# RazonIn4K/image-restoration-platform

Measured on AMD Instinct MI355X. Metric: restored images/sec @1024x1024 bs=8, higher is better.
Workload: dtype bf16; 1 GPU; 1024x1024 RGB u8, batch 8 per GPU: fused classifier scan + RestoreNet-v0 (43 convs, 779.9 GFLOP/image), seeded random-init weights; global_batch=8, parallelism=per-image data parallel x1, no collective, streams=1

## Files before the change

image_restoration_platform_amd/build.py:

```python
import concurrent.futures
import os
import subprocess
import sys

HERE = os.path.dirname(os.path.abspath(__file__))
CSRC = os.path.join(HERE, "csrc")
OBJ = os.path.join(HERE, "build")
LIB = os.path.join(HERE, "lib", "libire.so")

SOURCES = [
    ("classifier.hip", ["-ffp-contract=off"] + (["-DCLS_ABL=" + os.environ["CLS_ABL"]] if os.environ.get("CLS_ABL") else [])),
    ("conv_mfma.hip", []),
    ("conv_rb.hip", (["-DIRE_RB_ABLATE"] if os.environ.get("IRE_RB_ABLATE") else []) +
     (["-DIRE_RB_NGP64=" + os.environ["IRE_RB_NGP64"]] if os.environ.get("IRE_RB_NGP64") else [])),
    ("conv_w4.hip", (["-DIRE_W4_STAMPS"] if os.environ.get("IRE_RB_ABLATE") else []) +
     (["-DIRE_W4_TICKS"] if os.environ.get("IRE_RB_ABLATE") == "2" else []) +
     (["-DW4_TEPI=" + os.environ["IRE_W4_TEPI"]] if os.environ.get("IRE_W4_TEPI") else []) +
     (["-DIRE_W4_TL"] if os.environ.get("IRE_W4_TL") else [])),
    ("conv_up.hip", (["-DIRE_UP_ABL=" + os.environ["IRE_UP_ABL"]] if os.environ.get("IRE_UP_ABL") else []) +
     (["-DIRE_UP_D=" + os.environ["IRE_UP_D"]] if os.environ.get("IRE_UP_D") else []) +
     (["-DIRE_UP_TEPI=" + os.environ["IRE_UP_TEPI"]] if os.environ.get("IRE_UP_TEPI") else [])),
    ("conv_upq.hip", os.environ.get("UQ_DEFS", "").split()),
    ("conv_dnq.hip", os.environ.get("DQ_DEFS", "").split()),
    ("conv_down.hip", (["-DDN_LD_NT=" + os.environ["DN_LD_NT"]] if os.environ.get("DN_LD_NT") else [])),
    ("conv_stem.hip", []),
    ("conv_f8.hip", []),
    ("conv_pc.hip", (["-DC3_ABL=" + os.environ["C3_ABL"]] if os.environ.get("C3_ABL") else []) +
     (["-DC3_PRIO=" + os.environ["C3_PRIO"]] if os.environ.get("C3_PRIO") else []) +
     (["-DC3_RES_PRE=" + os.environ["C3_RES_PRE"]] if os.environ.get("C3_RES_PRE") else []) +
     (["-DC3_TEPI=" + os.environ["C3_TEPI"]] if os.environ.get("C3_TEPI") else []) +
     (["-DC3_TEPI64=" + os.environ["C3_TEPI64"]] if os.environ.get("C3_TEPI64") else []) +
     (["-DIRE_LD_ONCE32=" + os.environ["IRE_LD_ONCE32"]] if os.environ.get("IRE_LD_ONCE32") else []) +
     (["-DC3_PROD8=" + os.environ["C3_PROD8"]] if os.environ.get("C3_PROD8") else []) +
     (["-DIRE_PC_TICKS"] if os.environ.get("IRE_RB_ABLATE") == "2" else []) + (["-DIRE_W4_TL"] if os.environ.get("IRE_W4_TL") else [])),
    ("conv_pk.hip", (["-DPK_ABL=" + os.environ["PK_ABL"]] if os.environ.get("PK_ABL") else []) +
     (["-DPK_TICKS"] if os.environ.get("PK_TICKS") else []) + (["-DIRE_W4_TL"] if os.environ.get("IRE_W4_TL") else []) + os.environ.get("PK_DEFS", "").split()),
    ("gn.hip", []),
    ("fusion.hip", (["-DFUSE_FL=" + os.environ["FUSE_FL"]] if os.environ.get("FUSE_FL") else [])),
    ("preprocess.hip", []),
    ("encode.hip", []),
    ("deflate.hip", []),
    ("jpeg.hip", []),
    ("jpeg_progenc.hip", []),
    ("jpeg_dec.hip", []),
    ("png_dec.hip", []),
    ("icc.hip", []),
    ("codec.cpp", ["--offload-host-only"]),
    ("engine.cpp", []),
    ("strips.cpp", []),
    ("api.cpp", []),
]
COMMON = ["--offload-arch=gfx950", "-O3", "-std=c++17", "-fPIC", "-Wall", "-Wno-unused-function",
          "-D__HIP_PLATFORM_AMD__"] + ([] if os.environ.get("IRE_SLP") == "1" else ["-fno-slp-vectorize"]) + \
         (["-DIRE_ST_LINE=" + os.environ["IRE_ST_LINE"]] if os.environ.get("IRE_ST_LINE") else []) + \
         (["-DIRE_ST_PART=" + os.environ["IRE_ST_PART"]] if os.environ.get("IRE_ST_PART") else []) + \
         (["-DIRE_LD_ONCE=" + os.environ["IRE_LD_ONCE"]] if os.environ.get("IRE_LD_ONCE") else []) + \
         (["-DIRE_LD_IN=" + os.environ["IRE_LD_IN"]] if os.environ.get("IRE_LD_IN") else []) + \
         os.environ.get("IRE_XFLAGS", "").split()

def _hipcc():
    for c in (os.environ.get("HIPCC"), "/opt/rocm/bin/hipcc", "hipcc"):
        if c and (os.path.isabs(c) and os.path.exists(c) or not os.path.isabs(c)):
            return c
    raise RuntimeError("hipcc not found")


def _deps_mtime():
    m = 0.0
    for root, _, files in os.walk(CSRC):
        for f in files:
            if f.endswith((".hpp", ".inc", ".h")):
                m = max(m, os.path.getmtime(os.path.join(root, f)))
    m = max(m, os.path.getmtime(os.path.join(HERE, "..", "include", "ire.h")))
    return m


def _compile(src, extra, force, hdr_m):
    path = os.path.join(CSRC, src)
    obj = os.path.join(OBJ, src.replace(".", "_") + ".o")
    lang = ["-x", "hip"] if src.endswith((".hip", ".cpp")) else []
    cmd = [_hipcc()] + COMMON + extra + lang + ["-c", path, "-o", obj]
    stamp = obj + ".cmd"
    cmd_id = " ".join(cmd).replace(HERE, "<pkg>")
    same_cmd = os.path.exists(stamp) and open(stamp).read() == cmd_id
    if (not force and same_cmd and os.path.exists(obj) and os.path.getmtime(obj) > os.path.getmtime(path)
            and os.path.getmtime(obj) > hdr_m):
        return obj
    r = subprocess.run(cmd, capture_output=True, text=True)
    if r.returncode != 0:
        raise RuntimeError(f"hipcc failed for {src}:\n{r.stderr[-4000:]}")
    with open(stamp, "w") as f:
        f.write(cmd_id)
    return obj


def build(force=False, verbose=False):
    os.makedirs(OBJ, exist_ok=True)
    os.makedirs(os.path.dirname(LIB), exist_ok=True)
    srcs = [(s, f) for s, f in SOURCES if os.path.exists(os.path.join(CSRC, s))]
    if os.path.exists(os.path.join(CSRC, "fusion_stub.cpp")) and not os.path.exists(os.path.join(CSRC, "fusion.hip")):
        srcs.append(("fusion_stub.cpp", []))
    hdr_m = _deps_mtime()
    with concurrent.futures.ThreadPoolExecutor(max_workers=6) as ex:
        objs = list(ex.map(lambda sf: _compile(sf[0], sf[1], force, hdr_m), srcs))
    if force or not os.path.exists(LIB) or any(os.path.getmtime(o) > os.path.getmtime(LIB) for o in objs):
        cmd = [_hipcc(), "--offload-arch=gfx950", "-shared", "-fPIC", "-o", LIB] + objs + ["-lpthread"]
        r = subprocess.run(cmd, capture_output=True, text=True)
        if r.returncode != 0:
            raise RuntimeError(f"link failed:\n{r.stderr[-4000:]}")
    build_node_addon()
    try:
        build_torch_extension()
    except ImportError as e:
        print("build: torch extension skipped (%s)" % e, file=sys.stderr)
    except RuntimeError as e:
        print("build: torch extension NOT built: %s" % str(e)[-1500:], file=sys.stderr)
    if verbose:
        print("built", LIB)
    return LIB


def build_node_addon():
    src = os.path.join(HERE, "node", "ire_napi.cc")
    out = os.path.join(HERE, "node", "ire_napi.node")
    inc = "/usr/include/node"
    if not os.path.exists(os.path.join(inc, "node_api.h")):
        return None
    if os.path.exists(out) and os.path.getmtime(out) > max(os.path.getmtime(src), _deps_mtime()):
        return out
    r = subprocess.run(["g++", "-O2", "-shared", "-fPIC", "-I" + inc, "-DNODE_GYP_MODULE_NAME=ire_napi", src, "-o", out, "-ldl"],
                       capture_output=True, text=True)
    if r.returncode != 0:
        raise RuntimeError("node addon build failed:\n" + r.stderr[-2000:])
    return out


def build_torch_extension():
    src = os.path.join(CSRC, "torch_ext.cpp")
    out = os.path.join(HERE, "lib", "_ire_torch.so")
    import sysconfig
    from torch.utils import cpp_extension as ce
    incs = ce.include_paths() + [sysconfig.get_paths()["include"], "/opt/rocm/include"]
    libdir = ce.library_paths()[0]
    cmd = (["g++", "-O2", "-std=c++17", "-shared", "-fPIC", "-D__HIP_PLATFORM_AMD__", "-DUSE_ROCM", "-DTORCH_EXTENSION_NAME=_ire_torch",
            "-DTORCH_API_INCLUDE_EXTENSION_H", "-D_GLIBCXX_USE_CXX11_ABI=" + str(int(__import__("torch")._C._GLIBCXX_USE_CXX11_ABI))] +
           ["-isystem" + i for i in incs] + [src, "-o", out, "-L" + libdir, "-Wl,-rpath," + libdir,
            "-lc10", "-lc10_hip", "-ltorch_cpu", "-ltorch", "-ltorch_python", "-ldl"])
    stamp = os.path.join(OBJ, "_ire_torch.cmd")
    cmd_id = " ".join(cmd).replace(HERE, "<pkg>")
    if (os.path.exists(out) and os.path.exists(stamp) and open(stamp).read() == cmd_id and
            os.path.getmtime(out) > max(os.path.getmtime(src), os.path.getmtime(os.path.join(HERE, "..", "include", "ire.h")))):
        return out
    r = subprocess.run(cmd, capture_output=True, text=True)
    if r.returncode != 0:
        raise RuntimeError("torch extension build failed:\n" + r.stderr[-3000:])
    os.makedirs(OBJ, exist_ok=True)
    with open(stamp, "w") as f:
        f.write(cmd_id)
    return out


if __name__ == "__main__":
    build(force="--force" in sys.argv, verbose=True)
```

image_restoration_platform_amd/csrc/conv_pc.hip:

```cpp
#include "conv_mfma.hpp"
#include "conv_plan.hpp"
#include "conv_prims.hpp"
#include "gn_fold.hpp"
#include "persist.hpp"

#include <type_traits>

namespace ire {

namespace {

#ifndef C3_RES_PRE
#define C3_RES_PRE -1
#endif
#ifndef C3_SCALAR
#define C3_SCALAR 1
#endif
#ifndef C3_PRIO
#define C3_PRIO 1
#endif
#ifndef C3_TEPI
#define C3_TEPI 1
#endif
#ifndef IRE_LD_ONCE32
#define IRE_LD_ONCE32 2
#endif
#ifndef C3_TEPI64
#define C3_TEPI64 1
#endif
#ifndef C3_PROD8
#define C3_PROD8 0
#endif
#ifndef C3_INTERIOR
#define C3_INTERIOR 0
#endif
#ifndef C3_ABL
#define C3_ABL 0
#endif
constexpr int C3_CONS = 512, C3_PROD = 256, C3_THREADS = C3_CONS + C3_PROD;
constexpr int pc_prod(int C, bool head) { return (C3_PROD8 && C == 32 && !head) ? 512 : 256; }
constexpr int C3_TH = 16, C3_TW = 32, C3_IH = C3_TH + 2, C3_IW = C3_TW + 2;
constexpr int C3_IN_CHUNKS = C3_IH * C3_IW * 4;
constexpr int C3_P_ITERS = (C3_IN_CHUNKS + C3_PROD - 1) / C3_PROD;
constexpr int C3_IN_BYTES = C3_P_ITERS * C3_PROD * 16;
template <int C> struct PcCfg {
    static constexpr int NT = C < 64 ? 32 : 64;
    static constexpr int NBLK = C / NT;
    static constexpr int NKC = C / 32;
    static constexpr int NTL = NT / 32;
    static constexpr int W_STAGE = 36 * NT * 16;
    static constexpr int W_STAGE_CHUNKS = 36 * NT;
    static constexpr int W_LDS = NKC * W_STAGE;
    static constexpr int W_OFF = 2 * C3_IN_BYTES;
    static constexpr int BIAS_OFF = W_OFF + W_LDS;
    static constexpr int NCC = NT / 8;
    static constexpr int RED_OFF = BIAS_OFF + C * 4;
    static constexpr int RED_HALF = 8 * NCC * 4;
    static constexpr int COEF_IMGS = pc_coef_imgs(C);
    static constexpr int COEF_OFF = RED_OFF + 2 * RED_HALF * 4;
    static constexpr int HEAD_OFF = COEF_OFF + COEF_IMGS * C * 2 * 4;
    static constexpr int PATCH_OFF = HEAD_OFF + (C == 32 ? 8 * 2 * 2 * 96 : 0);
    static constexpr int CNT_OFF = PATCH_OFF + (C == 32 ? 8 * 2048 : 0);
    static constexpr int LDS = CNT_OFF + (C == 64 ? 16 : 0);
    static_assert(LDS <= 160 * 1024, "LDS");
};

template <int C, bool RESID, bool HEAD>
__global__ __launch_bounds__(C3_CONS + pc_prod(C, HEAD)) void conv_pc_kernel(ConvArgs a) {
    using K = PcCfg<C>;
    constexpr int PROD = pc_prod(C, HEAD), THREADS = C3_CONS + PROD;
    constexpr int P_ITERS = (C3_IN_CHUNKS + PROD - 1) / PROD;
    static_assert(P_ITERS * PROD * 16 == C3_IN_BYTES, "tile slots");
    constexpr int NKC = K::NKC, NTL = K::NTL, NCC = K::NCC, NT = K::NT;
    static_assert(!HEAD || C == 32, "the head is a C = 32 layer");
    __shared__ __attribute__((aligned(16))) unsigned char smem[K::LDS];
    const int tid = threadIdx.x;
    const int lane = tid & 63, wave = tid >> 6;
    const int r = lane & 31, h = lane >> 5;
    int stamp_item = 0;
    auto stamp = [&](int k) {
#ifdef IRE_PC_TICKS
        const unsigned long long t = __builtin_amdgcn_s_memtime();
        if (a.stamps && lane == 0 && (wave == 0 || wave == 8) && blockIdx.x < 8 && stamp_item < 64)
            a.stamps[(((size_t)blockIdx.x * 2 + (wave ? 1 : 0)) * 64 + stamp_item) * 10 + k] = t;
#else
        (void)k;
#endif
    };

    auto tl = [&](int slot) {
#ifdef IRE_W4_TL
        if (a.stamps && tid == 0) {
            a.stamps[(size_t)blockIdx.x * 32 + slot * 2] = __builtin_amdgcn_s_memrealtime();
            a.stamps[(size_t)blockIdx.x * 32 + slot * 2 + 1] = __builtin_amdgcn_s_memtime();
        }
#else
        (void)slot;
#endif
    };
    const int tiles_per_img = a.tiles_x * a.tiles_y;
    PersistCursor cursor(a.tiles_x, a.tiles_y, a.nimg, K::NBLK, NKC, (int)gridDim.x, (int)blockIdx.x, a.walk_rev != 0);
    const int n_items = cursor.my_items;
    if (n_items == 0) return;
    const int n_stages = n_items * NKC;
    tl(0);
    {
        const unsigned char* ws = reinterpret_cast<const unsigned char*>(a.w);
        const unsigned wl = (unsigned)(size_t)(__attribute__((address_space(3))) unsigned char*)smem + K::W_OFF;
        constexpr int PIECES = NKC * K::W_STAGE_CHUNKS / 64;
        static_assert((NKC * K::W_STAGE_CHUNKS) % 64 == 0, "whole wave-instructions");
        const int wv = __builtin_amdgcn_readfirstlane(wave);
        for (int p = wv; p < PIECES; p += THREADS / 64) glds16(ws + ((size_t)p * 64 + lane) * 16, wl + p * 1024);
    }
    if (a.gn_stats) gn_fold(a, smem, cursor.first_img, cursor.last_img, 512, reinterpret_cast<float2*>(smem + K::COEF_OFF));
    tl(1);

    {
        if (tid < C) reinterpret_cast<float*>(smem + K::BIAS_OFF)[tid] = a.bias[tid];
        if constexpr (C == 64) { if (tid == 0) *reinterpret_cast<unsigned*>(smem + K::CNT_OFF) = 0u; }
        const int nim = cursor.last_img - cursor.first_img + 1;
        const float2* ab = a.ab + (size_t)cursor.first_img * C;
        float2* cd = reinterpret_cast<float2*>(smem + K::COEF_OFF);
        if (!a.gn_stats) for (int i = tid; i < nim * C; i += THREADS) cd[i] = ab[i];
    }
    asm volatile("s_waitcnt vmcnt(0)" ::: "memory");
    __syncthreads();
    tl(2);

    if (__builtin_amdgcn_readfirstlane(wave) >= 8) {
#if C3_PRIO
        if (C3_PRIO != 1 || C != 32 || HEAD) asm volatile("s_setprio %0" :: "n"(C3_PRIO));
#endif
        const int tp = tid - C3_CONS;
        const int c8 = tp & 3;
        int rel[P_ITERS], lds_off[P_ITERS];
        unsigned pyx[P_ITERS];
#pragma unroll
        for (int i = 0; i < P_ITERS; ++i) {
            const int q = tp + i * PROD;
            const int p = q >> 2;
            const int py = p / C3_IW, px = p - py * C3_IW;
            pyx[i] = ((unsigned)py << 8) | (unsigned)px;
            rel[i] = (py * a.Win + px) * (2 * C) + c8 * 16;
            lds_off[i] = (p * 4 + (c8 ^ ((p >> 2) & 3))) * 16;
        }
        uint4 R[P_ITERS];
        unsigned okbits = 0;
        float cA[8], cB[8];
        PersistStage ls = cursor.cur;
        auto load_chunk = [&](int i) __attribute__((always_inline)) {
            const PersistItem& lit = ls.it;
            const int oy1 = lit.ty * C3_TH - 1, ox1 = lit.tx * C3_TW - 1;
            const char* base = reinterpret_cast<const char*>(a.in0) + (size_t)lit.img * a.in_rows * a.Win * (2 * C) + ls.kc * 64;
            const __amdgpu_buffer_rsrc_t irsrc = __builtin_amdgcn_make_buffer_rsrc(const_cast<char*>(base), 0, tensor_bytes(a.in_rows, a.Win, 2 * C) - (unsigned)(ls.kc * 64), 0x00020000);
            const unsigned base_off = (unsigned)((oy1 + a.in_row_off) * a.Win + ox1) * (unsigned)(2 * C);
            const int y_lo = max(a.iy_lo - oy1, 0), y_hi = min(a.iy_lo + a.iy_span - oy1, C3_IH);
            const int x_lo = max(-ox1, 0), x_hi = min(a.Win - ox1, C3_IW);
            const int py = (int)(pyx[i] >> 8), px = (int)(pyx[i] & 0xffu);
            const bool ok = (unsigned)(py - y_lo) < (unsigned)(y_hi - y_lo) && (unsigned)(px - x_lo) < (unsigned)(x_hi - x_lo);
            const unsigned off = ok ? base_off + rel[i] : 0xffffffffu;
            if constexpr (C3_ABL & 8) { R[i] = make_uint4(off, 0x3f803f80u, i, 0x3f803f80u); }
            else {
                const u32x4_t lv = __builtin_amdgcn_raw_buffer_load_b128(irsrc, off, 0, IRE_LD_IN);
                R[i] = make_uint4(lv.x, lv.y, lv.z, lv.w);
            }
            okbits = (okbits & ~(1u << i)) | (ok ? (1u << i) : 0u);
        };
        auto load_coeffs = [&](const PersistStage& st) __attribute__((always_inline)) {
            const float4* ab = reinterpret_cast<const float4*>(smem + K::COEF_OFF) + ((st.it.img - cursor.first_img) * C + st.kc * 32 + c8 * 8) / 2;
#pragma unroll
            for (int e = 0; e < 4; ++e) { const float4 v = ab[e]; cA[2 * e] = v.x; cB[2 * e] = v.y; cA[2 * e + 1] = v.z; cB[2 * e + 1] = v.w; }
        };
        auto transform_stage_v = [&](unsigned char* tile, auto interior_tag) __attribute__((always_inline)) {
            constexpr bool INTERIOR = decltype(interior_tag)::value;
            auto pair = [&](auto pp_tag) __attribute__((always_inline)) {
                constexpr int pp_ = decltype(pp_tag)::value, i = 2 * pp_;
                constexpr int NCH = i + 1 < P_ITERS ? 2 : 1;
                constexpr int NW = 4 * NCH, NV = 8 * NCH;
                constexpr int i1 = NCH == 2 ? i + 1 : i;
                const unsigned wds[8] = {R[i].x, R[i].y, R[i].z, R[i].w, R[i1].x, R[i1].y, R[i1].z, R[i1].w};
                unsigned o[8];
                if constexpr (C3_ABL & 1) {
#pragma unroll
                    for (int w = 0; w < NW; ++w) o[w] = wds[w];
                } else {
#if C3_SCALAR
                    float y[16], e[16];
#pragma unroll
                    for (int w = 0; w < NW; ++w) {
                        const int d = w & 3;
                        y[2 * w] = __builtin_fmaf(bf16_lo(wds[w]), cA[2 * d], cB[2 * d]);
                        y[2 * w + 1] = __builtin_fmaf(bf16_hi(wds[w]), cA[2 * d + 1], cB[2 * d + 1]);
                    }
#pragma unroll
                    for (int k = 0; k < NV; ++k) e[k] = y[k] * (-1.4426950408889634f);
                    __builtin_amdgcn_sched_barrier(0);
#pragma unroll
                    for (int k = 0; k < NV; ++k) e[k] = __builtin_amdgcn_exp2f(e[k]);
                    __builtin_amdgcn_sched_barrier(0);
#pragma unroll
                    for (int k = 0; k < NV; ++k) e[k] = e[k] + 1.0f;
                    __builtin_amdgcn_sched_barrier(0);
#pragma unroll
                    for (int k = 0; k < NV; ++k) e[k] = __builtin_amdgcn_rcpf(e[k]);
                    __builtin_amdgcn_sched_barrier(0);
#pragma unroll
                    for (int w = 0; w < NW; ++w) o[w] = pack_bf16(y[2 * w] * e[2 * w], y[2 * w + 1] * e[2 * w + 1]);
#else
                    static_assert(NCH == 2, "the packed-f32 form handles whole pairs");
                    f32x2_t y[8], e[8];
#pragma unroll
                    for (int w = 0; w < 8; ++w) {
                        const int d = w & 3;
                        const f32x2_t x = {bf16_lo(wds[w]), bf16_hi(wds[w])};
                        const f32x2_t A = {cA[2 * d], cA[2 * d + 1]}, B = {cB[2 * d], cB[2 * d + 1]};
                        y[w] = __builtin_elementwise_fma(x, A, B);
                        e[w] = y[w] * (-1.4426950408889634f);
                    }
                    __builtin_amdgcn_sched_barrier(0);
#pragma unroll
                    for (int w = 0; w < 8; ++w) e[w] = f32x2_t{__builtin_amdgcn_exp2f(e[w].x), __builtin_amdgcn_exp2f(e[w].y)};
                    __builtin_amdgcn_sched_barrier(0);
#pragma unroll
                    for (int w = 0; w < 8; ++w) e[w] = e[w] + 1.0f;
                    __builtin_amdgcn_sched_barrier(0);
#pragma unroll
                    for (int w = 0; w < 8; ++w) e[w] = f32x2_t{__builtin_amdgcn_rcpf(e[w].x), __builtin_amdgcn_rcpf(e[w].y)};
                    __builtin_amdgcn_sched_barrier(0);
#pragma unroll
                    for (int w = 0; w < 8; ++w) { const f32x2_t sv = y[w] * e[w]; o[w] = pack_bf16(sv.x, sv.y); }
#endif
                }
#pragma unroll
                for (int k = 0; k < NCH; ++k) {
                    uint4 ov = make_uint4(o[4 * k], o[4 * k + 1], o[4 * k + 2], o[4 * k + 3]);
                    if constexpr (!INTERIOR) {
                        const unsigned m = (okbits >> (i + k)) & 1u ? 0xffffffffu : 0u;
                        ov = make_uint4(o[4 * k] & m, o[4 * k + 1] & m, o[4 * k + 2] & m, o[4 * k + 3] & m);
                    }
                    *reinterpret_cast<uint4*>(tile + lds_off[i + k]) = ov;
                }
                load_chunk(i);
                if constexpr (NCH == 2) load_chunk(i + 1);
                __builtin_amdgcn_sched_barrier(0);
            };
            pair(std::integral_constant<int, 0>{}); pair(std::integral_constant<int, 1>{}); pair(std::integral_constant<int, 2>{});
            if constexpr (P_ITERS > 6) { pair(std::integral_constant<int, 3>{}); pair(std::integral_constant<int, 4>{}); }
        };
        unsigned past_last = 0u;
        {
            const int q = tp + (P_ITERS - 1) * PROD;
            past_last = (q >> 2) >= C3_IH * C3_IW ? (1u << (P_ITERS - 1)) : 0u;
        }
        auto transform_stage = [&](unsigned char* tile) __attribute__((always_inline)) {
            if constexpr (C3_INTERIOR) {
                if (__builtin_amdgcn_ballot_w64((okbits | past_last) != (1u << P_ITERS) - 1u) == 0) { transform_stage_v(tile, std::true_type{}); return; }
            }
            transform_stage_v(tile, std::false_type{});
        };
#pragma unroll
        for (int i = 0; i < P_ITERS; ++i) load_chunk(i);
        load_coeffs(ls);
        ls = cursor.next();
        transform_stage(smem);
        lds_barrier();
        for (int t = 0; t < n_stages; ++t) {
            stamp_item = t / NKC;
            stamp(3 * (t % NKC) + 0);
            load_coeffs(ls);
            ls = cursor.next();
            transform_stage(smem + ((t + 1) & 1) * C3_IN_BYTES);
            stamp(3 * (t % NKC) + 1);
            lds_barrier();
            stamp(3 * (t % NKC) + 2);
        }
        return;
    }

    int a_off[2][9];
#pragma unroll
    for (int m = 0; m < 2; ++m)
#pragma unroll
        for (int tap = 0; tap < 9; ++tap) {
            const int ky = tap / 3, kx = tap - ky * 3;
            const int p = (wave * 2 + m + ky) * C3_IW + r + kx;
            a_off[m][tap] = (p * 4 + (h ^ ((p >> 2) & 3))) * 16;
        }
    const unsigned char* wb = smem + K::W_OFF + (h * NT + r) * 16;
    const float* bias_lds = reinterpret_cast<const float*>(smem + K::BIAS_OFF);
    f32x16_t bias_acc;
    if constexpr (C == 32) {
#pragma unroll
        for (int i = 0; i < 16; ++i) bias_acc[i] = bias_lds[16 * (i >> 3) + 8 * h + (i & 7)];
    }
    float* red_base = reinterpret_cast<float*>(smem + K::RED_OFF);
    int st_img = -1, st_tile = 0, st_nb = 0, st_par = 0, red_par = 0;
    auto flush_stats = [&]() {
        if (HEAD || st_img < 0) return;
        constexpr int G = C / 8, NGL = NT / G, CPG = G / 8;
        if (tid < NGL) {
            const float* red = red_base + st_par * K::RED_HALF;
            float s = 0.f, q = 0.f;
#pragma unroll
            for (int w = 0; w < 8; ++w) {
                if constexpr (C == 32) {
                    const float* d = red + (w * NCC + (tid >> 1)) * 4 + 2 * (tid & 1);
                    s += d[0]; q += d[1];
                } else {
#pragma unroll
                    for (int k = 0; k < CPG; ++k) {
                        const float* d = red + (w * NCC + tid * CPG + k) * 4;
                        s += d[0] + d[2]; q += d[1] + d[3];
                    }
                }
            }
            float* st = a.stats + (((size_t)st_img * tiles_per_img + st_tile) * 8 + (st_nb * NT) / G + tid) * 2;
            st[0] = s; st[1] = q;
        }
        st_img = -1;
    };

    f32x16_t acc[2][NTL];
    uint4 erv[2 * NTL][2];
    constexpr int RES_WANT = C3_RES_PRE >= 0 ? C3_RES_PRE : (C == 64 ? 1 : 2);
    constexpr int RES_PRE = RES_WANT < 2 * NTL ? RES_WANT : 2 * NTL;
    unsigned eoffs[2];
    bool einb[2];
    constexpr bool TEPI = C3_TEPI && C == 32 && !HEAD;
    constexpr bool TEPI64 = C3_TEPI64 && C == 64 && !HEAD;
    unsigned toffs[2];
    bool trow[2];
    int tcol = 0;
    unsigned hin[2] = {0u, 0u};
    size_t hoff[2] = {0, 0};
    bool hok[2] = {false, false};
    PersistStage cs = cursor.cur;
    int stage_no = 0;
    lds_barrier();
    for (int t = 0; t < n_items; ++t) {
        const PersistItem it = cs.it;
        stamp_item = t;
        stamp(0);
        flush_stats();
        {
            const int oyb = it.ty * C3_TH + wave * 2, ox = it.tx * C3_TW + r;
            const bool colok = ox < a.Wout;
            const int oxc = min(ox, a.Wout - 1);
#pragma unroll
            for (int m = 0; m < 2; ++m) {
                const int oy = oyb + m;
                einb[m] = colok && oy < a.Hout;
                eoffs[m] = ((unsigned)((min(oy, a.Hout - 1) * a.Wout + oxc) * C + it.nb * NT) << 1) + (unsigned)(h * 16);
            }
            if constexpr (TEPI || TEPI64) {
                constexpr int LPP = C / 8;
                tcol = it.tx * C3_TW + lane / LPP;
#pragma unroll
                for (int m = 0; m < 2; ++m) {
                    const int oy = oyb + m;
                    trow[m] = oy < a.Hout;
                    toffs[m] = ((unsigned)((min(oy, a.Hout - 1) * a.Wout + tcol) * C + 8 * (lane % LPP)) << 1);
                }
            }
            if constexpr (RESID && TEPI64 && !(C3_ABL & 64)) {
                char* rbase = const_cast<char*>(reinterpret_cast<const char*>(a.resid)) + (size_t)it.img * a.Hout * a.Wout * (2 * C);
                const __amdgpu_buffer_rsrc_t rrsrc = __builtin_amdgcn_make_buffer_rsrc(rbase, 0, tensor_bytes(a.Hout, a.Wout, 2 * C), 0x00020000);
#pragma unroll
                for (int m = 0; m < 2; ++m)
#pragma unroll
                    for (int k = 0; k < RES_PRE; ++k) {
                        const bool ok = trow[m] && tcol + 8 * k < a.Wout;
                        const u32x4_t v = __builtin_amdgcn_raw_buffer_load_b128(rrsrc, ok ? toffs[m] + (unsigned)(8 * k * 2 * C) : 0xffffffffu, 0, IRE_LD_ONCE32);
                        erv[k][m] = make_uint4(v.x, v.y, v.z, v.w);
                    }
            } else
            if constexpr (RESID && TEPI && !(C3_ABL & 64)) {
                char* rbase = const_cast<char*>(reinterpret_cast<const char*>(a.resid)) + (size_t)it.img * a.Hout * a.Wout * (2 * C);
                const __amdgpu_buffer_rsrc_t rrsrc = __builtin_amdgcn_make_buffer_rsrc(rbase, 0, tensor_bytes(a.Hout, a.Wout, 2 * C), 0x00020000);
#pragma unroll
                for (int m = 0; m < 2; ++m)
#pragma unroll
                    for (int k = 0; k < 2; ++k) {
                        const bool ok = trow[m] && tcol + 16 * k < a.Wout;
                        const u32x4_t v = __builtin_amdgcn_raw_buffer_load_b128(rrsrc, ok ? toffs[m] + (unsigned)(16 * k * 2 * C) : 0xffffffffu, 0, IRE_LD_ONCE);
                        erv[k][m] = make_uint4(v.x, v.y, v.z, v.w);
                    }
            } else if constexpr (RESID && (C3_ABL & 64)) {
#pragma unroll
                for (int g = 0; g < 2 * NTL; ++g)
#pragma unroll
                    for (int m = 0; m < 2; ++m) erv[g][m] = make_uint4(eoffs[m], g, 0x3f803f80u, m);
            } else if constexpr (RESID) {
                const char* rbase = reinterpret_cast<const char*>(a.resid) + (size_t)it.img * a.Hout * a.Wout * (2 * C);
#pragma unroll
                for (int m = 0; m < 2; ++m)
#pragma unroll
                    for (int g = 0; g < RES_PRE; ++g) erv[g][m] = *reinterpret_cast<const uint4*>(rbase + eoffs[m] + (unsigned)(g * 32));
            }
            if constexpr (HEAD) {
                const int vbytes = 3 * min(C3_TW, a.Wout - it.tx * C3_TW);
#pragma unroll
                for (int m = 0; m < 2; ++m) {
                    const int oy = oyb + m;
                    hok[m] = oy < a.Hout && 4 * lane < vbytes;
                    hoff[m] = (((size_t)it.img * a.Hout + min(oy, a.Hout - 1)) * a.Wout + it.tx * C3_TW) * 3 + 4 * (size_t)min(lane, 23);
                    hin[m] = hok[m] ? *reinterpret_cast<const unsigned*>(a.u8_in + hoff[m]) : 0u;
                }
            }
        }
        if constexpr (C != 32) {
#pragma unroll
            for (int j = 0; j < NTL; ++j)
#pragma unroll
                for (int q = 0; q < 4; ++q) {
                    const float4 bv = *reinterpret_cast<const float4*>(bias_lds + it.nb * NT + j * 32 + 16 * (q >> 1) + 8 * h + 4 * (q & 1));
#pragma unroll
                    for (int m = 0; m < 2; ++m) { acc[m][j][4 * q + 0] = bv.x; acc[m][j][4 * q + 1] = bv.y; acc[m][j][4 * q + 2] = bv.z; acc[m][j][4 * q + 3] = bv.w; }
                }
        }
#pragma unroll NKC <= 2 ? NKC : 1
        for (int kc = 0; kc < NKC; ++kc) {
          auto stage_body = [&](auto par_tag) __attribute__((always_inline)) {
            constexpr int PAR = decltype(par_tag)::value;
            const int par = PAR >= 0 ? PAR : (stage_no & 1);
            const unsigned char* ib = smem + par * C3_IN_BYTES;
            const unsigned char* wk = wb + kc * K::W_STAGE;
            bf16x8_t af[2][2], bf[2][NTL];
            auto read_k = [&](int g, bf16x8_t (&pa)[2], bf16x8_t (&pw)[NTL]) __attribute__((always_inline)) {
                const int tap = g >> 1, cp = g & 1;
#pragma unroll
                for (int m = 0; m < 2; ++m) pa[m] = __builtin_bit_cast(bf16x8_t, *reinterpret_cast<const uint4*>(ib + (a_off[m][tap] ^ (cp << 5))));
#pragma unroll
                for (int j = 0; j < NTL; ++j) pw[j] = __builtin_bit_cast(bf16x8_t, *reinterpret_cast<const uint4*>(wk + ((tap * 4 + 2 * cp) * NT + j * 32) * 16));
            };
            read_k(0, af[0], bf[0]);
            if constexpr (!(C3_ABL & 4))
#pragma unroll
            for (int g = 0; g < 18; ++g) {
                if (g + 1 < 18) read_k(g + 1, af[(g + 1) & 1], bf[(g + 1) & 1]);
                __builtin_amdgcn_sched_barrier(0);
#pragma unroll
                for (int m = 0; m < 2; ++m)
#pragma unroll
                    for (int j = 0; j < NTL; ++j) {
                        if constexpr (C == 32) acc[m][j] = __builtin_amdgcn_mfma_f32_32x32x16_bf16(bf[g & 1][j], af[g & 1][m], (kc == 0 && g == 0) ? bias_acc : acc[m][j], 0, 0, 0);
                        else acc[m][j] = __builtin_amdgcn_mfma_f32_32x32x16_bf16(bf[g & 1][j], af[g & 1][m], acc[m][j], 0, 0, 0);
                    }
                __builtin_amdgcn_sched_barrier(0);
            }
          };
            if constexpr (NKC == 1 && HEAD) { if (stage_no & 1) stage_body(std::integral_constant<int, 1>{}); else stage_body(std::integral_constant<int, 0>{}); }
            else if constexpr (NKC == 2) { if (kc & 1) stage_body(std::integral_constant<int, 1>{}); else stage_body(std::integral_constant<int, 0>{}); }
            else stage_body(std::integral_constant<int, -1>{});
            ++stage_no;
            stamp(kc == 0 ? 1 : 3);
            if (kc + 1 < NKC) { cs = cursor.next(); lds_barrier(); stamp(2); }
        }
        if constexpr (RESID && TEPI64 && RES_PRE < 2 * NTL) {
            char* rbase = const_cast<char*>(reinterpret_cast<const char*>(a.resid)) + (size_t)it.img * a.Hout * a.Wout * (2 * C);
            const __amdgpu_buffer_rsrc_t rrsrc = __builtin_amdgcn_make_buffer_rsrc(rbase, 0, tensor_bytes(a.Hout, a.Wout, 2 * C), 0x00020000);
#pragma unroll
            for (int m = 0; m < 2; ++m)
#pragma unroll
                for (int k = RES_PRE; k < 2 * NTL; ++k) {
                    const bool ok = trow[m] && tcol + 8 * k < a.Wout;
                    const u32x4_t v = __builtin_amdgcn_raw_buffer_load_b128(rrsrc, ok ? toffs[m] + (unsigned)(8 * k * 2 * C) : 0xffffffffu, 0, 0);
                    erv[k][m] = make_uint4(v.x, v.y, v.z, v.w);
                }
        } else if constexpr (RESID && RES_PRE < 2 * NTL) {
            const char* rbase = reinterpret_cast<const char*>(a.resid) + (size_t)it.img * a.Hout * a.Wout * (2 * C);
#pragma unroll
            for (int m = 0; m < 2; ++m)
#pragma unroll
                for (int g = RES_PRE; g < 2 * NTL; ++g) erv[g][m] = *reinterpret_cast<const uint4*>(rbase + eoffs[m] + (unsigned)(g * 32));
        }
        if constexpr (HEAD) {
            unsigned char* hp = smem + K::HEAD_OFF + wave * (2 * 2 * 96);
#pragma unroll
            for (int m = 0; m < 2; ++m)
                if (lane < 24) *reinterpret_cast<unsigned*>(hp + m * 96 + 4 * lane) = hin[m];
#pragma unroll
            for (int m = 0; m < 2; ++m) {
                if (h == 0) {
#pragma unroll
                    for (int c = 0; c < 3; ++c) {
                        float vv = (float)hp[m * 96 + 3 * r + c] + acc[m][0][c];
                        vv = fminf(fmaxf(vv, 0.f), 255.f);
                        hp[192 + m * 96 + 3 * r + c] = (unsigned char)(int)floorf(vv + 0.5f);
                    }
                }
            }
#pragma unroll
            for (int m = 0; m < 2; ++m)
                if (hok[m]) *reinterpret_cast<unsigned*>(a.u8_out + hoff[m]) = *reinterpret_cast<const unsigned*>(hp + 192 + m * 96 + 4 * min(lane, 23));
        } else if constexpr (C3_ABL & 2) {
#pragma unroll
            for (int m = 0; m < 2; ++m)
#pragma unroll
                for (int j = 0; j < NTL; ++j) asm volatile("" :: "v"(acc[m][j]));
        } else if constexpr (TEPI64) {
            char* obase = reinterpret_cast<char*>(a.out) + (size_t)it.img * a.Hout * a.Wout * (2 * C);
            const __amdgpu_buffer_rsrc_t orsrc = __builtin_amdgcn_make_buffer_rsrc(obase, 0, tensor_bytes(a.Hout, a.Wout, 2 * C), 0x00020000);
            const bf16x2_t ones = __builtin_bit_cast(bf16x2_t, 0x3f803f80u);
            float* redw = red_base + red_par * K::RED_HALF;
            {
                volatile unsigned* cnt = reinterpret_cast<volatile unsigned*>(smem + K::CNT_OFF);
                asm volatile("s_waitcnt lgkmcnt(0)" ::: "memory");
                if (lane == 0) __hip_atomic_fetch_add(const_cast<unsigned*>(cnt), 1u, __ATOMIC_RELAXED, __HIP_MEMORY_SCOPE_WORKGROUP);
                const unsigned target = 8u * (unsigned)(t + 1);
                while ((unsigned)__builtin_amdgcn_readfirstlane((int)*cnt) < target) __builtin_amdgcn_s_sleep(1);
            }
            unsigned char* patch = smem + C3_IN_BYTES + wave * 4096;
            const int wsw = r & 7;
            const int pq = lane >> 3, cq = lane & 7;
            float sA = 0.f, qA = 0.f;
#pragma unroll
            for (int half = 0; half < 2; ++half)
#pragma unroll
            for (int m = 0; m < 2; ++m) {
#pragma unroll
                for (int g = 0; g < 2 * NTL; ++g) {
                    const f32x16_t& c = acc[m][g >> 1];
                    const int pp = g & 1;
                    const u32x4_t wv = {pack_bf16(c[8 * pp + 0], c[8 * pp + 1]), pack_bf16(c[8 * pp + 2], c[8 * pp + 3]),
                                        pack_bf16(c[8 * pp + 4], c[8 * pp + 5]), pack_bf16(c[8 * pp + 6], c[8 * pp + 7])};
                    *reinterpret_cast<u32x4_t*>(patch + r * 128 + (((2 * g + h) ^ wsw) << 4)) = wv;
                }
#pragma unroll
                for (int k = 2 * half; k < 2 * half + 2; ++k) {
                    const int p = pq + 8 * k;
                    const u32x4_t v = *reinterpret_cast<const u32x4_t*>(patch + p * 128 + ((cq ^ (p & 7)) << 4));
                    unsigned w[4] = {v.x, v.y, v.z, v.w};
                    if constexpr (RESID) {
                        const uint4 rr = erv[k][m];
                        const unsigned rw[4] = {rr.x, rr.y, rr.z, rr.w};
#pragma unroll
                        for (int d = 0; d < 4; ++d) w[d] = pack_bf16(bf16_lo(w[d]) + bf16_lo(rw[d]), bf16_hi(w[d]) + bf16_hi(rw[d]));
                    }
                    const bool ok = trow[m] && tcol + 8 * k < a.Wout;
                    const float mf = ok ? 1.f : 0.f;
                    float ts0 = 0.f, tq0 = 0.f;
                    if constexpr (!(C3_ABL & 32))
#pragma unroll
                    for (int d = 0; d < 4; ++d) {
                        const bf16x2_t bv = __builtin_bit_cast(bf16x2_t, w[d]);
                        ts0 = __builtin_amdgcn_fdot2_f32_bf16(bv, ones, ts0, false); tq0 = __builtin_amdgcn_fdot2_f32_bf16(bv, bv, tq0, false);
                    }
                    sA = __builtin_fmaf(ts0, mf, sA); qA = __builtin_fmaf(tq0, mf, qA);
                    const u32x4_t o4 = {w[0], w[1], w[2], w[3]};
                    if constexpr (C3_ABL & 16) asm volatile("" :: "v"(o4));
                    else __builtin_amdgcn_raw_buffer_store_b128(o4, orsrc, ok ? toffs[m] + (unsigned)(8 * k * 2 * C) : 0xffffffffu, 0, IRE_ST_LINE);
                }
            }
            if constexpr (!(C3_ABL & 32)) {
                float t2[2] = {sA, qA};
#pragma unroll
                for (int k = 0; k < 2; ++k) t2[k] = ror_add<8>(t2[k]);
#pragma unroll
                for (int k = 0; k < 2; ++k) t2[k] = swap16_add(t2[k]);
#pragma unroll
                for (int k = 0; k < 2; ++k) t2[k] = swap32_add(t2[k]);
                if (lane < 8) *reinterpret_cast<float4*>(redw + (wave * NCC + lane) * 4) = make_float4(t2[0], t2[1], 0.f, 0.f);
            }
            st_img = it.img; st_tile = it.tile; st_nb = it.nb; st_par = red_par; red_par ^= 1;
        } else if constexpr (TEPI) {
            char* obase = reinterpret_cast<char*>(a.out) + (size_t)it.img * a.Hout * a.Wout * (2 * C);
            const __amdgpu_buffer_rsrc_t orsrc = __builtin_amdgcn_make_buffer_rsrc(obase, 0, tensor_bytes(a.Hout, a.Wout, 2 * C), 0x00020000);
            const bf16x2_t ones = __builtin_bit_cast(bf16x2_t, 0x3f803f80u);
            float* redw = red_base + red_par * K::RED_HALF;
            unsigned char* patch = smem + K::PATCH_OFF + wave * 2048;
            const int wsw = (r >> 1) & 3;
            const int pq = lane >> 2, cq = lane & 3;
            float sA = 0.f, qA = 0.f, sB = 0.f, qB = 0.f;
#pragma unroll
            for (int m = 0; m < 2; ++m) {
                const f32x16_t& c = acc[m][0];
#pragma unroll
                for (int pp = 0; pp < 2; ++pp) {
                    const u32x4_t wv = {pack_bf16(c[8 * pp + 0], c[8 * pp + 1]), pack_bf16(c[8 * pp + 2], c[8 * pp + 3]),
                                        pack_bf16(c[8 * pp + 4], c[8 * pp + 5]), pack_bf16(c[8 * pp + 6], c[8 * pp + 7])};
                    *reinterpret_cast<u32x4_t*>(patch + r * 64 + (((2 * pp + h) ^ wsw) << 4)) = wv;
                }
#pragma unroll
                for (int k = 0; k < 2; ++k) {
                    const int p = pq + 16 * k;
                    const u32x4_t v = *reinterpret_cast<const u32x4_t*>(patch + p * 64 + ((cq ^ ((p >> 1) & 3)) << 4));
                    unsigned w[4] = {v.x, v.y, v.z, v.w};
                    if constexpr (RESID) {
                        const uint4 rr = erv[k][m];
                        const unsigned rw[4] = {rr.x, rr.y, rr.z, rr.w};
#pragma unroll
                        for (int d = 0; d < 4; ++d) w[d] = pack_bf16(bf16_lo(w[d]) + bf16_lo(rw[d]), bf16_hi(w[d]) + bf16_hi(rw[d]));
                    }
                    const bool ok = trow[m] && tcol + 16 * k < a.Wout;
                    const float mf = ok ? 1.f : 0.f;
                    float ts0 = 0.f, tq0 = 0.f, ts1 = 0.f, tq1 = 0.f;
                    if constexpr (!(C3_ABL & 32))
#pragma unroll
                    for (int d = 0; d < 4; ++d) {
                        const bf16x2_t bv = __builtin_bit_cast(bf16x2_t, w[d]);
                        if (d < 2) { ts0 = __builtin_amdgcn_fdot2_f32_bf16(bv, ones, ts0, false); tq0 = __builtin_amdgcn_fdot2_f32_bf16(bv, bv, tq0, false); }
                        else { ts1 = __builtin_amdgcn_fdot2_f32_bf16(bv, ones, ts1, false); tq1 = __builtin_amdgcn_fdot2_f32_bf16(bv, bv, tq1, false); }
                    }
                    sA = __builtin_fmaf(ts0, mf, sA); qA = __builtin_fmaf(tq0, mf, qA);
                    sB = __builtin_fmaf(ts1, mf, sB); qB = __builtin_fmaf(tq1, mf, qB);
                    const u32x4_t o4 = {w[0], w[1], w[2], w[3]};
                    if constexpr (C3_ABL & 16) asm volatile("" :: "v"(o4));
                    else __builtin_amdgcn_raw_buffer_store_b128(o4, orsrc, ok ? toffs[m] + (unsigned)(16 * k * 2 * C) : 0xffffffffu, 0, IRE_ST_LINE);
                }
            }
            if constexpr (!(C3_ABL & 32)) {
                float t4[4] = {sA, qA, sB, qB};
#pragma unroll
                for (int k = 0; k < 4; ++k) t4[k] = ror_add<4>(t4[k]);
#pragma unroll
                for (int k = 0; k < 4; ++k) t4[k] = ror_add<8>(t4[k]);
#pragma unroll
                for (int k = 0; k < 4; ++k) t4[k] = swap16_add(t4[k]);
#pragma unroll
                for (int k = 0; k < 4; ++k) t4[k] = swap32_add(t4[k]);
                if (lane < 4) *reinterpret_cast<float4*>(redw + (wave * NCC + lane) * 4) = make_float4(t4[0], t4[1], t4[2], t4[3]);
            }
            st_img = it.img; st_tile = it.tile; st_nb = it.nb; st_par = red_par; red_par ^= 1;
        } else {
            char* obase = reinterpret_cast<char*>(a.out) + (size_t)it.img * a.Hout * a.Wout * (2 * C);
            const __amdgpu_buffer_rsrc_t orsrc = __builtin_amdgcn_make_buffer_rsrc(obase, 0, tensor_bytes(a.Hout, a.Wout, 2 * C), 0x00020000);
            const bf16x2_t ones = __builtin_bit_cast(bf16x2_t, 0x3f803f80u);
            float* redw = red_base + red_par * K::RED_HALF;
            const float mf[2] = {einb[0] ? 1.f : 0.f, einb[1] ? 1.f : 0.f};
            float vs[4], vq[4];
#pragma unroll
            for (int j = 0; j < NTL; ++j)
#pragma unroll
            for (int pp = 0; pp < 2; ++pp) {
                const int g = 2 * j + pp;
                float sA = 0.f, qA = 0.f, sB = 0.f, qB = 0.f;
#pragma unroll
                for (int m = 0; m < 2; ++m) {
                    const f32x16_t& c = acc[m][j];
                    unsigned w[4] = {pack_bf16(c[8 * pp + 0], c[8 * pp + 1]), pack_bf16(c[8 * pp + 2], c[8 * pp + 3]),
                                     pack_bf16(c[8 * pp + 4], c[8 * pp + 5]), pack_bf16(c[8 * pp + 6], c[8 * pp + 7])};
                    if constexpr (RESID) {
                        const uint4 rr = erv[g][m];
                        const unsigned rw[4] = {rr.x, rr.y, rr.z, rr.w};
#pragma unroll
                        for (int d = 0; d < 4; ++d) w[d] = pack_bf16(bf16_lo(w[d]) + bf16_lo(rw[d]), bf16_hi(w[d]) + bf16_hi(rw[d]));
                    }
                    float ts0 = 0.f, tq0 = 0.f, ts1 = 0.f, tq1 = 0.f;
                    if constexpr (!(C3_ABL & 32))
#pragma unroll
                    for (int d = 0; d < 4; ++d) {
                        const bf16x2_t wv = __builtin_bit_cast(bf16x2_t, w[d]);
                        if (d < 2 || C != 32) { ts0 = __builtin_amdgcn_fdot2_f32_bf16(wv, ones, ts0, false); tq0 = __builtin_amdgcn_fdot2_f32_bf16(wv, wv, tq0, false); }
                        else { ts1 = __builtin_amdgcn_fdot2_f32_bf16(wv, ones, ts1, false); tq1 = __builtin_amdgcn_fdot2_f32_bf16(wv, wv, tq1, false); }
                    }
                    sA = __builtin_fmaf(ts0, mf[m], sA); qA = __builtin_fmaf(tq0, mf[m], qA);
                    if constexpr (C == 32) { sB = __builtin_fmaf(ts1, mf[m], sB); qB = __builtin_fmaf(tq1, mf[m], qB); }
                    const u32x4_t wv4 = {w[0], w[1], w[2], w[3]};
                    if constexpr (C3_ABL & 16) asm volatile("" :: "v"(wv4));
                    else __builtin_amdgcn_raw_buffer_store_b128(wv4, orsrc, einb[m] ? eoffs[m] + (unsigned)(g * 32) : 0xffffffffu, 0, IRE_ST_PART);
                }
                if constexpr (C == 32) { vs[2 * pp] = sA; vq[2 * pp] = qA; vs[2 * pp + 1] = sB; vq[2 * pp + 1] = qB; }
                else { vs[g] = sA; vq[g] = qA; }
            }
            if constexpr (!(C3_ABL & 32)) {
                const bool b0 = lane & 1, b1 = lane & 2;
                auto xch = [&](float keep, float give, auto ctrl_tag) __attribute__((always_inline)) -> float {
                    const int gg = __builtin_amdgcn_update_dpp(0, __builtin_bit_cast(int, give), decltype(ctrl_tag)::value, 0xf, 0xf, false);
                    return keep + __builtin_bit_cast(float, gg);
                };
                float u[4], t2[2];
#pragma unroll
                for (int k = 0; k < 4; ++k) u[k] = xch(b0 ? vq[k] : vs[k], b0 ? vs[k] : vq[k], std::integral_constant<int, 0xb1>{});
#pragma unroll
                for (int k = 0; k < 2; ++k) t2[k] = xch(b1 ? u[2 + k] : u[k], b1 ? u[k] : u[2 + k], std::integral_constant<int, 0x4e>{});
                t2[0] = ror_add<4>(t2[0]); t2[1] = ror_add<4>(t2[1]);
                t2[0] = ror_add<8>(t2[0]); t2[1] = ror_add<8>(t2[1]);
                t2[0] = swap16_add(t2[0]); t2[1] = swap16_add(t2[1]);
                if ((lane & 28) == 0) {
                    if constexpr (C == 32) {
                        float* d = redw + (wave * NCC + (b1 ? 2 : 0) + h) * 4 + (b0 ? 1 : 0);
                        d[0] = t2[0]; d[2] = t2[1];
                    } else {
                        float* d = redw + (wave * NCC + (b1 ? 4 : 0) + h) * 4 + (b0 ? 1 : 0);
                        d[0] = t2[0]; d[8] = t2[1];
                        d[2] = 0.f; d[10] = 0.f;
                    }
                }
            }
            st_img = it.img; st_tile = it.tile; st_nb = it.nb; st_par = red_par; red_par ^= 1;
        }
        stamp(NKC == 1 ? 3 : 4);
        cs = cursor.next();
        lds_barrier();
        stamp(5);
        tl(3 + (t < 8 ? t : 8));
    }
    flush_stats();
    tl(12);
}

}

void conv_pc_launch(bool resid, bool head, const ConvArgs& a, hipStream_t stream) {
    const int C = a.cout;
    if ((C != 32 && C != 64) || a.cin0 != C || a.nkc != C / 32 || a.nblocks != 1 || !a.ab)
        fail(IRE_ERR_INTERNAL, "internal: conv_pc arguments");
    if (head ? (C != 32 || !a.u8_in || !a.u8_out) : !a.stats) fail(IRE_ERR_INTERNAL, "internal: conv_pc arguments");
    const int items = a.tiles_x * a.tiles_y * a.nimg * a.nblocks;
    const int cus = persistent_grid_cus();
    if (!coef_table_fits(pc_coef_imgs(C), (long long)a.tiles_x * a.tiles_y, a.nimg, cus)) fail(IRE_ERR_INTERNAL, "internal: conv_pc batch");
    const int grid = persistent_grid(items, cus);
#define PC_GO(CC, RS, HD) hipLaunchKernelGGL((conv_pc_kernel<CC, RS, HD>), dim3(grid), dim3(C3_CONS + pc_prod(CC, HD)), 0, stream, a)
    if (head) PC_GO(32, false, true);
    else if (C == 32) { if (resid) PC_GO(32, true, false); else PC_GO(32, false, false); }
    else { if (resid) PC_GO(64, true, false); else PC_GO(64, false, false); }
#undef PC_GO
    IRE_HIP(hipGetLastError());
}

}
```

Before: 1124 images/sec.

## Reuse overlapping halo rows between vertically adjacent tiles in persistent conv producer

Reorders the producer slot-to-chunk mapping so the two halo rows shared by vertically adjacent tiles sit in one slot per thread. When the next persistent work item is the tile directly below (or above, on a reverse walk), that slot is copied from the other LDS buffer instead of being reloaded from global memory and re-transformed, and its global load is skipped. This trades a small amount of LDS copy and a restructured producer loop for fewer global loads and fewer GN/SiLU transform operations. It also changes the loop bound and adds a trailing barrier, which shifts the pipeline's stage accounting.

Result: no change. 1131 images/sec, median of 6 (+0.6%).

```diff
diff --git a/image_restoration_platform_amd/build.py b/image_restoration_platform_amd/build.py
--- a/image_restoration_platform_amd/build.py
+++ b/image_restoration_platform_amd/build.py
@@ -32,6 +32,7 @@
      (["-DC3_TEPI64=" + os.environ["C3_TEPI64"]] if os.environ.get("C3_TEPI64") else []) +
      (["-DIRE_LD_ONCE32=" + os.environ["IRE_LD_ONCE32"]] if os.environ.get("IRE_LD_ONCE32") else []) +
      (["-DC3_PROD8=" + os.environ["C3_PROD8"]] if os.environ.get("C3_PROD8") else []) +
+     (["-DC3_HALO=" + os.environ["C3_HALO"]] if os.environ.get("C3_HALO") else []) +
      (["-DIRE_PC_TICKS"] if os.environ.get("IRE_RB_ABLATE") == "2" else []) + (["-DIRE_W4_TL"] if os.environ.get("IRE_W4_TL") else [])),
     ("conv_pk.hip", (["-DPK_ABL=" + os.environ["PK_ABL"]] if os.environ.get("PK_ABL") else []) +
      (["-DPK_TICKS"] if os.environ.get("PK_TICKS") else []) + (["-DIRE_W4_TL"] if os.environ.get("IRE_W4_TL") else []) + os.environ.get("PK_DEFS", "").split()),
diff --git a/image_restoration_platform_amd/csrc/conv_pc.hip b/image_restoration_platform_amd/csrc/conv_pc.hip
--- a/image_restoration_platform_amd/csrc/conv_pc.hip
+++ b/image_restoration_platform_amd/csrc/conv_pc.hip
@@ -2,6 +2,7 @@
 #include "conv_plan.hpp"
 #include "conv_prims.hpp"
 #include "gn_fold.hpp"
+#include "halo_slots.hpp"
 #include "persist.hpp"
 
 #include <type_traits>
@@ -33,6 +34,9 @@
 #endif
 #ifndef C3_INTERIOR
 #define C3_INTERIOR 0
+#endif
+#ifndef C3_HALO
+#define C3_HALO 2
 #endif
 #ifndef C3_ABL
 #define C3_ABL 0
@@ -43,6 +47,7 @@
 constexpr int C3_IN_CHUNKS = C3_IH * C3_IW * 4;
 constexpr int C3_P_ITERS = (C3_IN_CHUNKS + C3_PROD - 1) / C3_PROD;
 constexpr int C3_IN_BYTES = C3_P_ITERS * C3_PROD * 16;
+static_assert(C3_IH == HALO_IH && C3_IW == HALO_IW && C3_IN_CHUNKS == HALO_CHUNKS && C3_PROD == HALO_THREADS && C3_P_ITERS == HALO_SLOTS, "halo_slots.hpp");
 template <int C> struct PcCfg {
     static constexpr int NT = C < 64 ? 32 : 64;
     static constexpr int NBLK = C / NT;
@@ -133,11 +138,13 @@
 #endif
         const int tp = tid - C3_CONS;
         const int c8 = tp & 3;
+        constexpr bool HALO = C3_HALO && C == 32 && PROD == HALO_THREADS;
+        const bool walk_rev = a.walk_rev != 0;
         int rel[P_ITERS], lds_off[P_ITERS];
         unsigned pyx[P_ITERS];
 #pragma unroll
         for (int i = 0; i < P_ITERS; ++i) {
-            const int q = tp + i * PROD;
+            const int q = HALO ? halo_slot_chunk(tp, i, walk_rev) : tp + i * PROD;
             const int p = q >> 2;
             const int py = p / C3_IW, px = p - py * C3_IW;
             pyx[i] = ((unsigned)py << 8) | (unsigned)px;
@@ -148,7 +155,7 @@
         unsigned okbits = 0;
         float cA[8], cB[8];
         PersistStage ls = cursor.cur;
-        auto load_chunk = [&](int i) __attribute__((always_inline)) {
+        auto load_chunk = [&](int i, bool skip = false) __attribute__((always_inline)) {
             const PersistItem& lit = ls.it;
             const int oy1 = lit.ty * C3_TH - 1, ox1 = lit.tx * C3_TW - 1;
             const char* base = reinterpret_cast<const char*>(a.in0) + (size_t)lit.img * a.in_rows * a.Win * (2 * C) + ls.kc * 64;
@@ -158,7 +165,7 @@
             const int x_lo = max(-ox1, 0), x_hi = min(a.Win - ox1, C3_IW);
             const int py = (int)(pyx[i] >> 8), px = (int)(pyx[i] & 0xffu);
             const bool ok = (unsigned)(py - y_lo) < (unsigned)(y_hi - y_lo) && (unsigned)(px - x_lo) < (unsigned)(x_hi - x_lo);
-            const unsigned off = ok ? base_off + rel[i] : 0xffffffffu;
+            const unsigned off = ok && !skip ? base_off + rel[i] : 0xffffffffu;
             if constexpr (C3_ABL & 8) { R[i] = make_uint4(off, 0x3f803f80u, i, 0x3f803f80u); }
             else {
                 const u32x4_t lv = __builtin_amdgcn_raw_buffer_load_b128(irsrc, off, 0, IRE_LD_IN);
@@ -171,11 +178,11 @@
 #pragma unroll
             for (int e = 0; e < 4; ++e) { const float4 v = ab[e]; cA[2 * e] = v.x; cB[2 * e] = v.y; cA[2 * e + 1] = v.z; cB[2 * e + 1] = v.w; }
         };
-        auto transform_stage_v = [&](unsigned char* tile, auto interior_tag) __attribute__((always_inline)) {
+        auto transform_stage_v = [&](unsigned char* tile, const unsigned char* other, bool reuse, bool skip0, auto interior_tag) __attribute__((always_inline)) {
             constexpr bool INTERIOR = decltype(interior_tag)::value;
-            auto pair = [&](auto pp_tag) __attribute__((always_inline)) {
-                constexpr int pp_ = decltype(pp_tag)::value, i = 2 * pp_;
-                constexpr int NCH = i + 1 < P_ITERS ? 2 : 1;
+            auto group = [&](auto i_tag, auto nch_tag, auto reload_tag) __attribute__((always_inline)) {
+                constexpr int i = decltype(i_tag)::value;
+                constexpr int NCH = decltype(nch_tag)::value;
                 constexpr int NW = 4 * NCH, NV = 8 * NCH;
                 constexpr int i1 = NCH == 2 ? i + 1 : i;
                 const unsigned wds[8] = {R[i].x, R[i].y, R[i].z, R[i].w, R[i1].x, R[i1].y, R[i1].z, R[i1].w};
@@ -240,40 +247,68 @@
                     }
                     *reinterpret_cast<uint4*>(tile + lds_off[i + k]) = ov;
                 }
-                load_chunk(i);
-                if constexpr (NCH == 2) load_chunk(i + 1);
+                if constexpr (decltype(reload_tag)::value) {
+                    load_chunk(i);
+                    if constexpr (NCH == 2) load_chunk(i + 1);
+                    __builtin_amdgcn_sched_barrier(0);
+                }
+            };
+            using One = std::integral_constant<int, 1>;
+            using Two = std::integral_constant<int, 2>;
+            auto pair = [&](auto i_tag) __attribute__((always_inline)) { group(i_tag, Two{}, std::true_type{}); };
+            if constexpr (HALO) {
+                if (reuse) {
+                    const uint4 v = *reinterpret_cast<const uint4*>(other + halo_src_delta(walk_rev) + lds_off[0]);
+                    *reinterpret_cast<uint4*>(tile + lds_off[0]) = v;
+                } else {
+                    group(std::integral_constant<int, 0>{}, One{}, std::false_type{});
+                }
+                load_chunk(0, C3_HALO >= 2 && skip0);
                 __builtin_amdgcn_sched_barrier(0);
-            };
-            pair(std::integral_constant<int, 0>{}); pair(std::integral_constant<int, 1>{}); pair(std::integral_constant<int, 2>{});
-            if constexpr (P_ITERS > 6) { pair(std::integral_constant<int, 3>{}); pair(std::integral_constant<int, 4>{}); }
+                pair(std::integral_constant<int, 1>{}); pair(std::integral_constant<int, 3>{}); pair(std::integral_constant<int, 5>{}); pair(std::integral_constant<int, 7>{});
+                group(std::integral_constant<int, 9>{}, One{}, std::true_type{});
+            } else {
+                pair(std::integral_constant<int, 0>{}); pair(std::integral_constant<int, 2>{});
+                if constexpr (P_ITERS > 6) {
+                    pair(std::integral_constant<int, 4>{}); pair(std::integral_constant<int, 6>{}); pair(std::integral_constant<int, 8>{});
+                } else {
+                    group(std::integral_constant<int, 4>{}, One{}, std::true_type{});
+                }
+            }
         };
         unsigned past_last = 0u;
         {
-            const int q = tp + (P_ITERS - 1) * PROD;
+            const int q = HALO ? halo_slot_chunk(tp, P_ITERS - 1, walk_rev) : tp + (P_ITERS - 1) * PROD;
             past_last = (q >> 2) >= C3_IH * C3_IW ? (1u << (P_ITERS - 1)) : 0u;
         }
-        auto transform_stage = [&](unsigned char* tile) __attribute__((always_inline)) {
+        auto transform_stage = [&](unsigned char* tile, const unsigned char* other, bool reuse, bool skip0) __attribute__((always_inline)) {
             if constexpr (C3_INTERIOR) {
-                if (__builtin_amdgcn_ballot_w64((okbits | past_last) != (1u << P_ITERS) - 1u) == 0) { transform_stage_v(tile, std::true_type{}); return; }
-            }
-            transform_stage_v(tile, std::false_type{});
+                if (__builtin_amdgcn_ballot_w64((okbits | past_last) != (1u << P_ITERS) - 1u) == 0) { transform_stage_v(tile, other, reuse, skip0, std::true_type{}); return; }
+            }
+            transform_stage_v(tile, other, reuse, skip0, std::false_type{});
         };
 #pragma unroll
         for (int i = 0; i < P_ITERS; ++i) load_chunk(i);
         load_coeffs(ls);
+        PersistItem staged = ls.it;
         ls = cursor.next();
-        transform_stage(smem);
+        bool reuse = false, reuse_next = HALO && halo_adjacent(staged, ls.it, walk_rev);
+        transform_stage(smem, smem + C3_IN_BYTES, reuse, reuse_next);
         lds_barrier();
-        for (int t = 0; t < n_stages; ++t) {
+        for (int t = 0; t + 1 < n_stages; ++t) {
             stamp_item = t / NKC;
             stamp(3 * (t % NKC) + 0);
             load_coeffs(ls);
+            reuse = reuse_next;
+            staged = ls.it;
             ls = cursor.next();
-            transform_stage(smem + ((t + 1) & 1) * C3_IN_BYTES);
+            reuse_next = HALO && halo_adjacent(staged, ls.it, walk_rev);
+            transform_stage(smem + ((t + 1) & 1) * C3_IN_BYTES, smem + (t & 1) * C3_IN_BYTES, reuse, reuse_next);
             stamp(3 * (t % NKC) + 1);
             lds_barrier();
             stamp(3 * (t % NKC) + 2);
         }
+        lds_barrier();
         return;
     }
 
diff --git a/image_restoration_platform_amd/csrc/halo_slots.hpp b/image_restoration_platform_amd/csrc/halo_slots.hpp
--- /dev/null
+++ b/image_restoration_platform_amd/csrc/halo_slots.hpp
@@ -0,0 +1,31 @@
+#pragma once
+
+#include "persist.hpp"
+
+namespace ire {
+
+constexpr int HALO_IH = 18, HALO_IW = 34;
+constexpr int HALO_CHUNKS = HALO_IH * HALO_IW * 4;
+constexpr int HALO_THREADS = 256, HALO_SLOTS = 10;
+constexpr int HALO_SHIFT = (HALO_IH - 2) * HALO_IW * 4;
+constexpr int HALO_SHIFT_BYTES = HALO_SHIFT * 16;
+
+IRE_HD int halo_slot_chunk(int tp, int i, bool reverse) {
+    if (!reverse) return tp + HALO_THREADS * i;
+    if (i == 0) return HALO_SHIFT + tp;
+    const int q = tp + HALO_THREADS * (i - 1);
+    return q < HALO_SHIFT ? q : q + HALO_THREADS;
+}
+
+IRE_HD int halo_lds_off(int q) {
+    const int p = q >> 2;
+    return (p * 4 + ((q & 3) ^ ((p >> 2) & 3))) * 16;
+}
+
+IRE_HD int halo_src_delta(bool reverse) { return reverse ? -HALO_SHIFT_BYTES : HALO_SHIFT_BYTES; }
+
+IRE_HD bool halo_adjacent(const PersistItem& prev, const PersistItem& cur, bool reverse) {
+    return cur.img == prev.img && cur.tx == prev.tx && cur.ty == prev.ty + (reverse ? -1 : 1);
+}
+
+}
```
